# yaramohamadi/Pairwise_Sample_Optimization

Measured on AMD Instinct MI355X. Metric: PSO train-step imgs/sec (paired 1024² SDXL) at 1/2/4/8 MI355X, higher is better.
Workload: dtype bf16; 1 GPU; C2: SDXL-Turbo PSO train step, LoRA r=32 grads, 2 pairs/GPU/micro-step, gas 2, 2-step sampler (T=1); global_batch=4, seq_len=4096, resolution=1024, parallelism=dp1, launch=eager

## Files before the change

### include/pso_amd.h

```cpp
#ifndef PSO_AMD_H
#define PSO_AMD_H

#include <stddef.h>
#include <stdint.h>

#ifdef __cplusplus
extern "C" {
#endif

#define PSO_ABI_VERSION 1

#define PSO_OK 0
#define PSO_ERR_ARG 1
#define PSO_ERR_HIP 2
#define PSO_ERR_UNSUPPORTED 3

#define PSO_F32 0
#define PSO_BF16 1
#define PSO_F16 2
#define PSO_U8 2

#define PSO_MODE_TURBO 0
#define PSO_MODE_DMD 1
#define PSO_MODE_DMD_F16 2
// ... 120 lines not shown
                      long sdq_b, void* dk, long lddk, long sdk_b, void* dv, long lddv, long sdv_b, void* ws,
                      size_t ws_bytes, void* stream);

int pso_geglu_fwd(long M, int F, const void* in, long ldi, void* out, long ldo, void* stream);
int pso_geglu_bwd(long M, int F, const void* in, long ldi, const void* dout, long lddo, void* din, long lddi,
                  void* stream);
int pso_silu(long n, const void* x, void* y, void* stream);
int pso_timestep_embedding(int n, int dim, const float* t, void* out, long ldo, int out_col, void* stream);
int pso_transpose(int R, int Rp, int C, const void* in, long ldi, void* out, long ldo, void* stream);
int pso_im2col3(int B, int H, int W, int C, const void* in, void* out, int Kp, void* stream);

int pso_colsum_acc(long M, int N, const void* x, long ldx, long rows_per_group, float* out, long ldo, void* stream);
int pso_layer_norm_dparam(int M, int C, const void* x, long ldx, const void* dy, long lddy, const float* stats,
                          float* dgamma, float* dbeta, void* stream);
size_t pso_colsum_acc_ws_bytes(long M, int N, long rows_per_group);
int pso_colsum_acc_ws(long M, int N, const void* x, long ldx, long rows_per_group, float* out, long ldo, void* ws,
                      size_t ws_bytes, void* stream);
size_t pso_layer_norm_dparam_ws_bytes(int M, int C);
int pso_layer_norm_dparam_ws(int M, int C, const void* x, long ldx, const void* dy, long lddy, const float* stats,
                             float* dgamma, float* dbeta, void* ws, size_t ws_bytes, void* stream);
int pso_im2col_conv(int mode, int B, const void* src1, int C1, const void* src2, int C2, int H, int W, int Ho, int Wo,
                    int stride, int pad, void* out, long ldo, void* stream);
int pso_sumpool2(int B, int H, int W, int C, const void* in, const void* dadd, void* out, void* stream);
int pso_axpby(long n, float a, const void* x, float b, const void* z, void* y, void* stream);
int pso_cast_f32_bf16(long n, const float* x, float scale, void* y, void* stream);
int pso_cast_bf16_f32(long n, const void* x, float* y, void* stream);
int pso_conv_weight_t(int Co, int ks, int Ci, int flip, const void* w, void* wt, void* stream);
int pso_transpose_batched(int n, const void* descs, int max_r, int max_c, void* stream);
int pso_lora_pack(int n, const void* descs, long max_items, float scale, void* stream);
int pso_lora_grad_fold(int n, const void* descs, long max_items, void* stream);
int pso_transpose_multi(int n, const void* descs, int total_tiles, void* stream);
int pso_gather_rows(long n, long row_bytes, const void* src, const int64_t* idx, void* dst, void* stream);
int pso_nchw_to_nhwc(int B, int C, int Cp, long HW, const void* src, int src_dtype, float scale, void* dst,
                     void* stream);
int pso_softmax_rows(int M, int N, void* x, long ld, void* stream);
int pso_nhwc_to_nchw(int B, int C, long HW, const void* src, void* dst, int dst_dtype, void* stream);
int pso_concat_channels(long npix, int C1, const void* x1, int C2, const void* x2, void* out, void* stream);
int pso_split_channels(long npix, int C1, int C2, const void* in, void* y1, void* y2, const void* add2,
                       void* stream);

size_t pso_grad_clip_ws_bytes(long n);
int pso_grad_clip_coef(long n, const float* grad, float grad_scale, float max_norm, float* out_norm_coef, void* ws,
                       size_t ws_bytes, void* stream);
int pso_adamw_step(long n, float* param, const float* grad, float* exp_avg, float* exp_avg_sq, float lr, float beta1,
                   float beta2, float eps, float weight_decay, int step, float grad_scale, const float* clip_coef,
                   void* stream);
size_t pso_adamw8bit_blocks(long n);
void pso_adamw8bit_maps(float* signed_map, float* unsigned_map);
int pso_adamw8bit_step(long n, float* param, const float* grad, uint8_t* exp_avg_q, uint8_t* exp_avg_sq_q,
                       float* absmax_m, float* absmax_v, float lr, float beta1, float beta2, float eps,
                       float weight_decay, int step, float grad_scale, const float* clip_coef, void* stream);
int pso_adamw8bit_step_bf16(long n, float* param, void* param_bf16, const float* grad, uint8_t* exp_avg_q,
                            uint8_t* exp_avg_sq_q, float* absmax_m, float* absmax_v, float lr, float beta1, float beta2,
                            float eps, float weight_decay, int step, float grad_scale, const float* clip_coef,
                            void* stream);
int pso_adamw8bit_step_blocks(long n, int nblk, const long* desc, float* param, void* param_bf16, const float* grad,
                              uint8_t* exp_avg_q, uint8_t* exp_avg_sq_q, float* absmax_m, float* absmax_v,
                              float* exp_avg_32, float* exp_avg_sq_32, float lr, float beta1, float beta2, float eps,
                              float weight_decay, int step, float grad_scale, const float* clip_coef, void* stream);
int pso_adamw8bit_step_blocks_zero_grad(long n, int nblk, const long* desc, float* param, void* param_bf16,
                                        float* grad, uint8_t* exp_avg_q, uint8_t* exp_avg_sq_q, float* absmax_m,
                                        float* absmax_v, float* exp_avg_32, float* exp_avg_sq_32, float lr,
// ... 76 lines not shown
```

### pairwise_sample_optimization_amd/_lib.py

```python
import ctypes
import os

import torch

_HERE = os.path.dirname(os.path.abspath(__file__))
KNOBS = os.environ.get("PSO_LIB", "") == "knobs"
F16 = os.environ.get("PSO_LIB", "") == "f16"
LIB_PATH = os.environ.get("PSO_LIB_PATH") or os.path.join(
    _HERE, "libpso_amd_knobs.so" if KNOBS else "libpso_amd_f16.so" if F16 else "libpso_amd.so")

PSO_F32 = 0
PSO_BF16 = 1
PSO_F16 = 2
ELEM_DTYPE = torch.float16 if F16 else torch.bfloat16
ELEM_CODE = PSO_F16 if F16 else PSO_BF16
MODE_TURBO = 0
MODE_DMD = 1
MODE_DMD_F16 = 2
MODE_DMD_BF16 = 3
COEF_STRIDE = 8
AMP_WORDS = 16
(AMP_SCALE, AMP_INV_SCALE, AMP_FOUND_INF, AMP_GROWTH_TRACKER, AMP_STEP, AMP_SKIPPED, AMP_NORM, AMP_CLIP_COEF,
 AMP_GRAD_MUL, AMP_BC1, AMP_BC2_SQRT, AMP_C1, AMP_C2) = range(13)
AMP_INT_WORDS = (AMP_FOUND_INF, AMP_GROWTH_TRACKER, AMP_STEP, AMP_SKIPPED)
# ... 68 lines not shown
    "pso_group_norm_ws_bytes": (csz, [ci, ci, ci]),
    "pso_group_norm_fwd": (ci, [ci, ci, ci, ci, cf, vp, vp, vp, ci, vp, vp, vp, csz, vp]),
    "pso_group_norm_bwd": (ci, [ci, ci, ci, ci, vp, vp, vp, vp, vp, ci, vp, vp, vp, vp, ci, vp, csz, vp]),
    "pso_layer_norm_fwd": (ci, [ci, ci, cf, vp, cl, vp, vp, vp, cl, vp, vp]),
    "pso_layer_norm_bwd": (ci, [ci, ci, vp, cl, vp, cl, vp, vp, vp, cl, vp, cl, vp]),
    "pso_attention_fwd": (ci, [ci, ci, ci, ci, vp, cl, cl, vp, cl, cl, vp, cl, cl, cf, vp, cl, cl, vp, vp]),
    "pso_attention_bwd_ws_bytes": (csz, [ci, ci, ci, ci]),
    "pso_attention_bwd": (ci, [ci, ci, ci, ci, vp, cl, cl, vp, cl, cl, vp, cl, cl, vp, cl, cl, vp, vp, cl, cl, cf,
                               vp, cl, cl, vp, cl, cl, vp, cl, cl, vp, csz, vp]),
    "pso_geglu_fwd": (ci, [cl, ci, vp, cl, vp, cl, vp]),
    "pso_geglu_bwd": (ci, [cl, ci, vp, cl, vp, cl, vp, cl, vp]),
    "pso_silu": (ci, [cl, vp, vp, vp]),
    "pso_timestep_embedding": (ci, [ci, ci, vp, vp, cl, ci, vp]),
    "pso_transpose": (ci, [ci, ci, ci, vp, cl, vp, cl, vp]),
    "pso_im2col3": (ci, [ci, ci, ci, ci, vp, vp, ci, vp]),
    "pso_colsum_acc": (ci, [cl, ci, vp, cl, cl, vp, cl, vp]),
    "pso_layer_norm_dparam": (ci, [ci, ci, vp, cl, vp, cl, vp, vp, vp, vp]),
    "pso_colsum_acc_ws_bytes": (csz, [cl, ci, cl]),
    "pso_colsum_acc_ws": (ci, [cl, ci, vp, cl, cl, vp, cl, vp, csz, vp]),
    "pso_layer_norm_dparam_ws_bytes": (csz, [ci, ci]),
    "pso_layer_norm_dparam_ws": (ci, [ci, ci, vp, cl, vp, cl, vp, vp, vp, vp, csz, vp]),
    "pso_im2col_conv": (ci, [ci, ci, vp, ci, vp, ci, ci, ci, ci, ci, ci, ci, vp, cl, vp]),
    "pso_sumpool2": (ci, [ci, ci, ci, ci, vp, vp, vp, vp]),
    "pso_axpby": (ci, [cl, cf, vp, cf, vp, vp, vp]),
    "pso_cast_f32_bf16": (ci, [cl, vp, cf, vp, vp]),
    "pso_cast_bf16_f32": (ci, [cl, vp, vp, vp]),
    "pso_conv_weight_t": (ci, [ci, ci, ci, ci, vp, vp, vp]),
    "pso_concat_channels": (ci, [cl, ci, vp, ci, vp, vp, vp]),
    "pso_nchw_to_nhwc": (ci, [ci, ci, ci, cl, vp, ci, cf, vp, vp]),
    "pso_softmax_rows": (ci, [ci, ci, vp, cl, vp]),
    "pso_grad_clip_ws_bytes": (csz, [cl]),
    "pso_transpose_batched": (ci, [ci, vp, ci, ci, vp]),
    "pso_transpose_multi": (ci, [ci, vp, ci, vp]),
    "pso_lora_pack": (ci, [ci, vp, cl, cf, vp]),
    "pso_lora_grad_fold": (ci, [ci, vp, cl, vp]),
    "pso_gather_rows": (ci, [cl, cl, vp, vp, vp, vp]),
    "pso_grad_clip_coef": (ci, [cl, vp, cf, cf, vp, vp, csz, vp]),
    "pso_adamw_step": (ci, [cl, vp, vp, vp, vp, cf, cf, cf, cf, cf, ci, cf, vp, vp]),
    "pso_adamw8bit_blocks": (csz, [cl]),
    "pso_adamw8bit_maps": (None, [vp, vp]),
    "pso_adamw8bit_step": (ci, [cl, vp, vp, vp, vp, vp, vp, cf, cf, cf, cf, cf, ci, cf, vp, vp]),
    "pso_adamw8bit_step_bf16": (ci, [cl, vp, vp, vp, vp, vp, vp, vp, cf, cf, cf, cf, cf, ci, cf, vp, vp]),
    "pso_adamw8bit_step_blocks": (ci, [cl, ci, vp, vp, vp, vp, vp, vp, vp, vp, vp, vp, cf, cf, cf, cf, cf, ci, cf,
                                       vp, vp]),
    "pso_adamw8bit_step_blocks_zero_grad": (ci, [cl, ci, vp, vp, vp, vp, vp, vp, vp, vp, vp, vp, cf, cf, cf, cf, cf,
                                                 ci, cf, vp, vp]),
    "pso_amp_unscale_clip": (ci, [cl, vp, cf, cf, cf, cf, vp, vp, csz, vp]),
    "pso_amp_update": (ci, [vp, cf, cf, ci, vp]),
    "pso_adamw_step_amp": (ci, [cl, vp, vp, vp, vp, cf, cf, cf, cf, cf, vp, vp]),
    "pso_adamw8bit_step_blocks_amp": (ci, [cl, ci, vp, vp, vp, vp, vp, vp, vp, vp, vp, vp, cf, cf, cf, cf, cf, vp,
                                           vp]),
# ... 114 lines not shown
```

### pairwise_sample_optimization_amd/csrc/elementwise.hip

```cpp
#include "common.h"

__device__ __forceinline__ void unpack8e(uint4 v, float* f) {
  const uint32_t w[4] = {v.x, v.y, v.z, v.w};
#pragma unroll
  for (int i = 0; i < 4; ++i) {
    f[2 * i] = bf2f(w[i] & 0xffff);
    f[2 * i + 1] = bf2f(w[i] >> 16);
  }
}
__device__ __forceinline__ uint4 pack8e(const float* f) {
  return make_uint4(pack2bf(f[0], f[1]), pack2bf(f[2], f[3]), pack2bf(f[4], f[5]), pack2bf(f[6], f[7]));
}

static int grid_for(long n, int per_thread = 1) {
  long g = (n / per_thread + 255) / 256;
  if (g > 8192) g = 8192;
  return (int)(g < 1 ? 1 : g);
}

#define GRID_STRIDE(i, n) for (long i = blockIdx.x * (long)blockDim.x + threadIdx.x; i < (n); i += (long)gridDim.x * blockDim.x)


__global__ void geglu_fwd_kernel(long M, int F, const bf16_t* __restrict__ in, long ldi, bf16_t* __restrict__ out,
                                 long ldo) {
// ... 128 lines not shown
  const int C8 = C / 8;
  GRID_STRIDE(v, (long)B * H * W * C8) {
    const long pix = v / C8;
    const int c = (int)(v - pix * C8) * 8;
    const int b = (int)(pix / ((long)H * W));
    const int rem = (int)(pix - (long)b * H * W);
    const int y = rem / W, x = rem - y * W;
    float acc[8] = {0, 0, 0, 0, 0, 0, 0, 0};
#pragma unroll
    for (int dy = 0; dy < 2; ++dy)
#pragma unroll
      for (int dx = 0; dx < 2; ++dx) {
        float a[8];
        unpack8e(*reinterpret_cast<const uint4*>(in + (((long)b * 2 * H + 2 * y + dy) * 2 * W + 2 * x + dx) * C + c), a);
#pragma unroll
        for (int j = 0; j < 8; ++j) acc[j] += a[j];
      }
    if (dadd) {
      float a[8];
      unpack8e(*reinterpret_cast<const uint4*>(dadd + pix * C + c), a);
#pragma unroll
      for (int j = 0; j < 8; ++j) acc[j] += a[j];
    }
    *reinterpret_cast<uint4*>(out + pix * C + c) = pack8e(acc);
  }
}

__global__ void axpby_kernel(long n8, float a, const bf16_t* __restrict__ x, float b, const bf16_t* __restrict__ z,
                             bf16_t* __restrict__ y) {
  GRID_STRIDE(v, n8) {
    float p[8], q[8];
    unpack8e(*reinterpret_cast<const uint4*>(x + v * 8), p);
    if (z) unpack8e(*reinterpret_cast<const uint4*>(z + v * 8), q);
#pragma unroll
    for (int j = 0; j < 8; ++j) p[j] = a * p[j] + (z ? b * q[j] : 0.f);
    *reinterpret_cast<uint4*>(y + v * 8) = pack8e(p);
  }
}

__global__ void cast_f32_bf16_kernel(long n, const float* __restrict__ x, float scale, bf16_t* __restrict__ y) {
  long done = 0;
  if (((reinterpret_cast<uintptr_t>(x) | reinterpret_cast<uintptr_t>(y)) & 15) == 0) {
    done = n & ~7L;
    GRID_STRIDE(v, n >> 3) {
      const float4 a = reinterpret_cast<const float4*>(x)[2 * v], b = reinterpret_cast<const float4*>(x)[2 * v + 1];
      reinterpret_cast<uint4*>(y)[v] = make_uint4(pack2bf(a.x * scale, a.y * scale), pack2bf(a.z * scale, a.w * scale),
// ... 39 lines not shown
      for (int e = 0; e < 8; ++e) tile[r][c + e] = (co < Co && ci + e < Ci) ? src[e] : (bf16_t)0;
    }
  }
  __syncthreads();
  const int lx = t & 63, ly = t >> 6;
  for (int i = ly; i < 64; i += 4) {
    const int ci = ci0 + i, co = co0 + lx;
    if (ci < Ci && co < Co) wt[((long)ci * ks * ks + tap2) * Co + co] = tile[lx][i];
  }
}

__global__ void concat_kernel(long npix, int C1, const bf16_t* __restrict__ x1, int C2, const bf16_t* __restrict__ x2,
                              bf16_t* __restrict__ out) {
  const int C8 = (C1 + C2) / 8, c18 = C1 / 8;
  GRID_STRIDE(v, npix * C8) {
    const long p = v / C8;
    const int ch = (int)(v - p * C8);
    const uint4 val = ch < c18 ? *reinterpret_cast<const uint4*>(x1 + p * C1 + ch * 8)
                               : *reinterpret_cast<const uint4*>(x2 + p * C2 + (ch - c18) * 8);
    *reinterpret_cast<uint4*>(out + v * 8) = val;
  }
}

__global__ void split_kernel(long npix, int C1, int C2, const bf16_t* __restrict__ in, bf16_t* __restrict__ y1,
                             bf16_t* __restrict__ y2, const bf16_t* __restrict__ add2) {
  const int C8 = (C1 + C2) / 8, c18 = C1 / 8;
  GRID_STRIDE(v, npix * C8) {
    const long p = v / C8;
    const int ch = (int)(v - p * C8);
    const uint4 val = *reinterpret_cast<const uint4*>(in + v * 8);
    if (ch < c18) {
      *reinterpret_cast<uint4*>(y1 + p * C1 + ch * 8) = val;
    } else {
      bf16_t* o = y2 + p * C2 + (ch - c18) * 8;
      if (add2) {
        float a[8], b[8];
        unpack8e(val, a);
        unpack8e(*reinterpret_cast<const uint4*>(add2 + p * C2 + (ch - c18) * 8), b);
#pragma unroll
        for (int j = 0; j < 8; ++j) a[j] += b[j];
        *reinterpret_cast<uint4*>(o) = pack8e(a);
      } else {
        *reinterpret_cast<uint4*>(o) = val;
      }
    }
  }
// ... 120 lines not shown
                     void* stream) {
  PSO_DTYPE_CHECK(src_dtype, "pso_nchw_to_nhwc");
  PSO_ARG_CHECK(src && dst && Cp >= C, "pso_nchw_to_nhwc: bad args");
  nchw_to_nhwc_kernel<<<grid_for((long)B * Cp * HW), 256, 0, (hipStream_t)stream>>>(
      B, C, Cp, HW, src, src_dtype == PSO_F32, scale, (bf16_t*)dst);
  return pso_check_launch("pso_nchw_to_nhwc");
}

int pso_nhwc_to_nchw(int B, int C, long HW, const void* src, void* dst, int dst_dtype, void* stream) {
  PSO_DTYPE_CHECK(dst_dtype, "pso_nhwc_to_nchw");
  PSO_ARG_CHECK(src && dst, "pso_nhwc_to_nchw: bad args");
  nhwc_to_nchw_kernel<<<grid_for((long)B * C * HW), 256, 0, (hipStream_t)stream>>>(B, C, HW, (const bf16_t*)src,
                                                                                  dst, dst_dtype == PSO_F32);
  return pso_check_launch("pso_nhwc_to_nchw");
}

int pso_concat_channels(long npix, int C1, const void* x1, int C2, const void* x2, void* out, void* stream) {
  PSO_ARG_CHECK(C1 % 8 == 0 && C2 % 8 == 0 && x1 && x2 && out, "pso_concat_channels: C %% 8");
  concat_kernel<<<grid_for(npix * (C1 + C2) / 8), 256, 0, (hipStream_t)stream>>>(
      npix, C1, (const bf16_t*)x1, C2, (const bf16_t*)x2, (bf16_t*)out);
  return pso_check_launch("pso_concat_channels");
}

int pso_split_channels(long npix, int C1, int C2, const void* in, void* y1, void* y2, const void* add2,
                       void* stream) {
  PSO_ARG_CHECK(C1 % 8 == 0 && C2 % 8 == 0 && in && y1 && y2, "pso_split_channels: C %% 8");
  split_kernel<<<grid_for(npix * (C1 + C2) / 8), 256, 0, (hipStream_t)stream>>>(
      npix, C1, C2, (const bf16_t*)in, (bf16_t*)y1, (bf16_t*)y2, (const bf16_t*)add2);
  return pso_check_launch("pso_split_channels");
}

int pso_geglu_fwd(long M, int F, const void* in, long ldi, void* out, long ldo, void* stream) {
  PSO_ARG_CHECK(F % 8 == 0 && ldi % 8 == 0 && ldo % 8 == 0 && in && out, "pso_geglu_fwd: bad args");
  geglu_fwd_kernel<<<grid_for(M * (F / 8)), 256, 0, (hipStream_t)stream>>>(M, F, (const bf16_t*)in, ldi,
                                                                          (bf16_t*)out, ldo);
  return pso_check_launch("pso_geglu_fwd");
}

int pso_geglu_bwd(long M, int F, const void* in, long ldi, const void* dout, long lddo, void* din, long lddi,
                  void* stream) {
  PSO_ARG_CHECK(F % 8 == 0 && ldi % 8 == 0 && lddo % 8 == 0 && lddi % 8 == 0 && in && dout && din,
                "pso_geglu_bwd: bad args");
  geglu_bwd_kernel<<<grid_for(M * (F / 8)), 256, 0, (hipStream_t)stream>>>(M, F, (const bf16_t*)in, ldi,
                                                                          (const bf16_t*)dout, lddo, (bf16_t*)din,
                                                                          lddi);
  return pso_check_launch("pso_geglu_bwd");
// ... 19 lines not shown
}

int pso_transpose(int R, int Rp, int C, const void* in, long ldi, void* out, long ldo, void* stream) {
  PSO_ARG_CHECK(in && out && Rp >= R, "pso_transpose: bad args");
  dim3 grid(cdiv(C, 64), cdiv(Rp, 64));
  transpose_kernel<<<grid, 256, 0, (hipStream_t)stream>>>(R, Rp, C, (const bf16_t*)in, ldi, (bf16_t*)out, ldo);
  return pso_check_launch("pso_transpose");
}

int pso_im2col3(int B, int H, int W, int C, const void* in, void* out, int Kp, void* stream) {
  PSO_ARG_CHECK(Kp >= 9 * C && in && out, "pso_im2col3: Kp < 9C");
  im2col3_kernel<<<grid_for((long)B * H * W * Kp), 256, 0, (hipStream_t)stream>>>(B, H, W, C, (const bf16_t*)in, 0,
                                                                                  (bf16_t*)out, Kp);
  return pso_check_launch("pso_im2col3");
}

int pso_sumpool2(int B, int H, int W, int C, const void* in, const void* dadd, void* out, void* stream) {
  PSO_ARG_CHECK(C % 8 == 0 && in && out, "pso_sumpool2: C %% 8");
  sumpool2_kernel<<<grid_for((long)B * H * W * C / 8), 256, 0, (hipStream_t)stream>>>(
      B, H, W, C, (const bf16_t*)in, (const bf16_t*)dadd, (bf16_t*)out);
  return pso_check_launch("pso_sumpool2");
}

int pso_axpby(long n, float a, const void* x, float b, const void* z, void* y, void* stream) {
  PSO_ARG_CHECK(n % 8 == 0 && x && y, "pso_axpby: n %% 8");
  axpby_kernel<<<grid_for(n / 8), 256, 0, (hipStream_t)stream>>>(n / 8, a, (const bf16_t*)x, b, (const bf16_t*)z,
                                                                 (bf16_t*)y);
  return pso_check_launch("pso_axpby");
}

int pso_cast_f32_bf16(long n, const float* x, float scale, void* y, void* stream) {
  cast_f32_bf16_kernel<<<grid_for(n, 8), 256, 0, (hipStream_t)stream>>>(n, x, scale, (bf16_t*)y);
  return pso_check_launch("pso_cast_f32_bf16");
}

int pso_cast_bf16_f32(long n, const void* x, float* y, void* stream) {
  cast_bf16_f32_kernel<<<grid_for(n, 8), 256, 0, (hipStream_t)stream>>>(n, (const bf16_t*)x, y);
  return pso_check_launch("pso_cast_bf16_f32");
}

int pso_conv_weight_t(int Co, int ks, int Ci, int flip, const void* w, void* wt, void* stream) {
  conv_weight_t_kernel<<<dim3(cdiv(Ci, 64), cdiv(Co, 64), ks * ks), 256, 0, (hipStream_t)stream>>>(
      Co, ks, Ci, flip, (const bf16_t*)w, (bf16_t*)wt);
  return pso_check_launch("pso_conv_weight_t");
}

// ... 2 lines not shown
```

### pairwise_sample_optimization_amd/kernels.py

```python
import ctypes
import math
import os

import torch

from . import _lib
from ._lib import check, lib, ptr, require_cuda, stream_ptr, dtype_code, PSO_BF16, PSO_F32

CONV_NORMAL, CONV_UP2, CONV_T2 = 1, 2, 3
ELEM = _lib.ELEM_DTYPE

PROFILE = None


def _prof_begin():
    if PROFILE is None:
        return None
    e0 = torch.cuda.Event(enable_timing=True)
    e0.record()
    return e0


def _prof_end(e0, flops, nbytes=0.0, tag=None):
    if e0 is not None:
# ... 293 lines not shown
        self.pending = {}


def conv2d(x, weight, *, x2=None, mode=CONV_NORMAL, stride=1, pad=None, out_hw=None, bias=None, rowbias=None,
           resid=None, a2=None, w2=None, alpha=1.0, out=None, out_dtype=ELEM, accumulate=False):
    require_cuda(x, weight)
    B, H, W, C1 = x.shape
    C2 = x2.shape[3] if x2 is not None else 0
    Cout, ks, ks2, Ct = weight.shape
    assert ks == ks2 and Ct == C1 + C2 and x.is_contiguous() and weight.is_contiguous()
    if pad is None:
        pad = ks // 2
    if out_hw is None:
        if mode == CONV_UP2:
            out_hw = (2 * H, 2 * W)
        elif mode == CONV_T2:
            out_hw = (2 * H, 2 * W)
        else:
            out_hw = ((H + 2 * pad - ks) // stride + 1, (W + 2 * pad - ks) // stride + 1)
    Ho, Wo = out_hw
    if out is None:
        out = torch.empty((B, Ho, Wo, Cout), device=x.device, dtype=out_dtype)
    K2 = a2.shape[1] if a2 is not None else 0
    o2 = out.view(B * Ho * Wo, -1) if out.is_contiguous() else None
    ldo = Cout if o2 is None else o2.stride(0)
    key = ("conv", B, Ho, Wo, Cout, ks * ks * Ct, K2)
    wsb = _GEMM_WS.get(key)
    if wsb is None:
        wsb = _GEMM_WS[key] = int(lib().pso_conv2d_ws_bytes(B, Ho, Wo, Cout, ks * ks * Ct, K2))
    args = (mode, B, ptr(x), C1, ptr(x2), C2, H, W, Ho, Wo, ks, stride, pad, ptr(weight), Cout,
            ptr(a2), _row_stride(a2) if a2 is not None else 0, K2,
            ptr(w2), _row_stride(w2) if w2 is not None else 0, float(alpha), ptr(bias),
            ptr(rowbias), rowbias.stride(0) if rowbias is not None else 0,
            ptr(resid), Cout if resid is not None else 0, ptr(out), ldo, dtype_code(out), int(accumulate))
    e0 = _prof_begin()
    if wsb:
        ws = torch.empty(wsb, device=x.device, dtype=torch.uint8)
        check(lib().pso_conv2d_ws(*args, ptr(ws), wsb, stream_ptr()), "pso_conv2d_ws")
    else:
        check(lib().pso_conv2d(*args, stream_ptr()), "pso_conv2d")
    _prof_end(e0, 2.0 * B * Ho * Wo * Cout * (ks * ks * (C1 + C2) + K2),
              2.0 * (B * H * W * (C1 + C2) + Cout * ks * ks * (C1 + C2) + B * Ho * Wo * K2 + Cout * K2)
              + out.element_size() * B * Ho * Wo * Cout, ("conv", mode, B, H, W, C1, C2, Cout, ks, stride, K2))
    return out


def step_logprob(mode, sample, eps, coef, prev=None, noise=None, noise_shared=False):
    require_cuda(sample, eps, coef, prev, noise)
# ... 270 lines not shown
        _row_stride(out)
        _TRANSPOSE_BATCH.append((x, out))
        return out
    check(lib().pso_transpose(R, Rp, C, ptr(x), _row_stride(x), ptr(out), _row_stride(out), stream_ptr()),
          "pso_transpose")
    return out


def im2col3(x, kp):
    B, H, W, C = x.shape
    out = torch.empty((B * H * W, kp), device=x.device, dtype=x.dtype)
    check(lib().pso_im2col3(B, H, W, C, ptr(x.contiguous()), ptr(out), kp, stream_ptr()), "pso_im2col3")
    return out


def sumpool2(x, dadd=None):
    B, H2, W2, C = x.shape
    out = torch.empty((B, H2 // 2, W2 // 2, C), device=x.device, dtype=x.dtype)
    check(lib().pso_sumpool2(B, H2 // 2, W2 // 2, C, ptr(x.contiguous()), ptr(dadd), ptr(out), stream_ptr()),
          "pso_sumpool2")
    return out


def axpby(a, x, b=0.0, z=None, out=None):
    out = torch.empty_like(x) if out is None else out
    check(lib().pso_axpby(x.numel(), float(a), ptr(x.contiguous()), float(b),
                          ptr(z.contiguous()) if z is not None else None, ptr(out), stream_ptr()), "pso_axpby")
    return out


_FULLGRAD_ATOMIC = os.environ.get("PSO_FULLGRAD_ATOMIC", "0") == "1"
_STREAM_WS = {}


def _stream_ws(nbytes, device):
    key = (device.index, torch.cuda.current_stream(device).cuda_stream)
    ws = _STREAM_WS.get(key)
    if ws is None or ws.numel() < nbytes:
        ws = _STREAM_WS[key] = torch.empty(max(int(nbytes * 1.25), 1 << 16), device=device, dtype=torch.uint8)
    return ws


def colsum_acc(x, out, rows_per_group=None):
    M, N = x.shape
    rpg = M if rows_per_group is None else rows_per_group
    if _FULLGRAD_ATOMIC:
# ... 44 lines not shown


def cast_bf16_f32(x, out=None):
    out = torch.empty(x.shape, device=x.device, dtype=torch.float32) if out is None else out
    check(lib().pso_cast_bf16_f32(x.numel(), ptr(x.contiguous()), ptr(out), stream_ptr()), "pso_cast_bf16_f32")
    return out


def conv_weight_t(w, flip):
    Co, ks, _, Ci = w.shape
    out = torch.empty((Ci, ks, ks, Co), device=w.device, dtype=w.dtype)
    check(lib().pso_conv_weight_t(Co, ks, Ci, int(flip), ptr(w.contiguous()), ptr(out), stream_ptr()),
          "pso_conv_weight_t")
    return out


def concat_channels(x1, x2):
    C1, C2 = x1.shape[-1], x2.shape[-1]
    out = torch.empty(x1.shape[:-1] + (C1 + C2,), device=x1.device, dtype=x1.dtype)
    npix = x1.numel() // C1
    check(lib().pso_concat_channels(npix, C1, ptr(x1.contiguous()), C2, ptr(x2.contiguous()), ptr(out),
                                    stream_ptr()), "pso_concat_channels")
    return out


def split_channels(x, C1, add2=None):
    C = x.shape[-1]
    C2 = C - C1
    y1 = torch.empty(x.shape[:-1] + (C1,), device=x.device, dtype=x.dtype)
    y2 = torch.empty(x.shape[:-1] + (C2,), device=x.device, dtype=x.dtype)
    npix = x.numel() // C
    check(lib().pso_split_channels(npix, C1, C2, ptr(x.contiguous()), ptr(y1), ptr(y2),
                                   ptr(add2.contiguous()) if add2 is not None else None, stream_ptr()),
          "pso_split_channels")
    return y1, y2


def nchw_to_nhwc(x, pad_to=None, scale=1.0):
    B, C, H, W = x.shape
    Cp = pad_to or C
    out = torch.empty((B, H, W, Cp), device=x.device, dtype=ELEM)
    check(lib().pso_nchw_to_nhwc(B, C, Cp, H * W, ptr(x.contiguous()), dtype_code(x), float(scale), ptr(out),
                                 stream_ptr()), "pso_nchw_to_nhwc")
    return out


# ... 450 lines not shown
```

### pairwise_sample_optimization_amd/unet.py

```python
import math
import os
from dataclasses import dataclass, field, replace
from types import SimpleNamespace

import torch
import torch.nn as nn

from . import _lib
from . import kernels as K

ELEM = _lib.ELEM_DTYPE
TN_BATCH = os.environ.get("PSO_TN_BATCH", "1") != "0"


@dataclass
class UNetConfig:
    in_channels: int = 4
    out_channels: int = 4
    block_out_channels: tuple = (320, 640, 1280)
    layers_per_block: int = 2
    transformer_layers_per_block: tuple = (1, 2, 10)
    down_has_attn: tuple = (False, True, True)
    head_dim: int = 64
    cross_attention_dim: int = 2048
# ... 740 lines not shown
        self.wt_int = K.transpose(self.w_int)
        self.out.prepare()

    def _remap(self):
        return {"net.0.proj": self.proj, "net.2": self.out}


class Transformer2DModel(nn.Module):

    def __init__(self, C, depth, cross_dim, groups):
        super().__init__()
        self.C, self.groups = C, groups
        self.norm = Norm(C)
        self.proj_in = Linear(C, C)
        self.transformer_blocks = nn.ModuleList([BasicTransformerBlock(C, cross_dim) for _ in range(depth)])
        self.proj_out = Linear(C, C)

    def prepare(self):
        self.proj_in.prepare()
        self.proj_out.prepare()
        for b in self.transformer_blocks:
            b.prepare()

    def fwd(self, x, rt, path):
        B, H, W, C = x.shape
        xn, st = K.group_norm_fwd(x, self.norm.weight, self.norm.bias, self.groups, 1e-6, False)
        h = K.gemm(xn.view(-1, C), self.proj_in.weight, bias=self.proj_in.bias)
        if rt.save:
            rt.saved.append({"x": rt.pol(x), "st": rt.pol(st), "xn": xn.view(-1, C) if rt.fg is not None else None})
        for i, blk in enumerate(self.transformer_blocks):
            h = blk.fwd(h, rt, f"{path}.transformer_blocks.{i}")
        if rt.save and rt.fg is not None:
            rt.saved.append({"hout": h})
        return K.gemm(h, self.proj_out.weight, bias=self.proj_out.bias, resid=x.view(-1, C)).view(B, H, W, C)

    def bwd(self, dy, rt, path, need_dx=True):
        B, H, W, C = dy.shape
        d2 = dy.view(-1, C)
        fg = rt.fg
        if fg is not None:
            _lin_dw(fg, self.proj_out, d2, rt.saved.pop()["hout"], rt)
        dh = K.gemm(d2, self.proj_out.wt)
        for i in reversed(range(len(self.transformer_blocks))):
            dh = self.transformer_blocks[i].bwd(dh, rt.saved.pop(), rt, f"{path}.transformer_blocks.{i}",
                                                need_dx=need_dx or i > 0)
        sv = rt.saved.pop()
        if not need_dx:
            return None
        dn = K.gemm(dh, self.proj_in.wt).view(B, H, W, C)
        if fg is not None:
            _lin_dw(fg, self.proj_in, dh, sv["xn"], rt)
            return K.group_norm_bwd(sv["x"], dn, sv["st"], self.norm.weight, self.norm.bias, False, dadd=dy,
                                    dgamma=fg.g(self.norm.weight), dbeta=fg.g(self.norm.bias), accumulate=True)
        return K.group_norm_bwd(sv["x"], dn, sv["st"], self.norm.weight, self.norm.bias, False, dadd=dy)


class ResnetBlock2D(nn.Module):
    def __init__(self, cin, cout, groups, eps, temb_dim):
        super().__init__()
        self.cin, self.cout, self.groups, self.eps = cin, cout, groups, eps
        self.norm1 = Norm(cin)
        self.conv1 = Conv2d(cin, cout, 3)
        self.time_emb_proj = Linear(temb_dim, cout) if temb_dim else None
        self.norm2 = Norm(cout)
        self.conv2 = Conv2d(cout, cout, 3)
        self.conv_shortcut = Conv2d(cin, cout, 1) if cin != cout else None

    def prepare(self):
        self.conv1.prepare()
        self.conv2.prepare()
        if self.conv_shortcut is not None:
            self.conv_shortcut.prepare()

    def fwd(self, x, rt, temb=None):
        h1, st1 = K.group_norm_fwd(x, self.norm1.weight, self.norm1.bias, self.groups, self.eps, True)
        c1 = K.conv2d(h1, self.conv1.w_nhwc, bias=self.conv1.bias, rowbias=temb)
        h2, st2 = K.group_norm_fwd(c1, self.norm2.weight, self.norm2.bias, self.groups, self.eps, True)
        if self.conv_shortcut is not None:
            B, H, W, _ = x.shape
            sc = K.gemm(x.view(-1, self.cin), self.conv_shortcut.w_mat, bias=self.conv_shortcut.bias)
            sc = sc.view(B, H, W, self.cout)
        else:
            sc = x
        out = K.conv2d(h2, self.conv2.w_nhwc, bias=self.conv2.bias, resid=sc)
        if rt.save:
            sv = {"x": rt.pol(x), "st1": rt.pol(st1), "c1": rt.pol(c1), "st2": rt.pol(st2)}
            if rt.fg is not None:
                sv.update(h1=h1, h2=h2)
            rt.saved.append(sv)
        return out

    def bwd(self, dout, rt):
        sv = rt.saved.pop()
        fg = rt.fg
        B, H, W, _ = dout.shape
        dh2 = K.conv2d(dout, self.conv2.w_dx)
        if fg is not None:
            _conv_dw(fg, self.conv2, dout.view(-1, self.cout), sv["h2"], rt, K.im2col_conv)
            dc1 = K.group_norm_bwd(sv["c1"], dh2, sv["st2"], self.norm2.weight, self.norm2.bias, True,
                                   dgamma=fg.g(self.norm2.weight), dbeta=fg.g(self.norm2.bias), accumulate=True)
            dc2 = dc1.view(-1, self.cout)
            _conv_dw(fg, self.conv1, dc2, sv["h1"], rt, K.im2col_conv)
            K.colsum_acc(dc2, rt.dtemb[:, self._temb_off:self._temb_off + self.cout], rows_per_group=H * W)
        else:
            dc1 = K.group_norm_bwd(sv["c1"], dh2, sv["st2"], self.norm2.weight, self.norm2.bias, True)
        dh1 = K.conv2d(dc1, self.conv1.w_dx)
        if self.conv_shortcut is not None:
# ... 23 lines not shown
        self.conv.prepare()

    def fwd(self, x, rt):
        if rt.save:
            rt.saved.append({"hw": x.shape[1:3], "x": x if rt.fg is not None else None})
        return K.conv2d(x, self.conv.w_nhwc, stride=2, bias=self.conv.bias)

    def bwd(self, dy, rt):
        sv = rt.saved.pop()
        if rt.fg is not None:
            _conv_dw(rt.fg, self.conv, dy.reshape(-1, self.conv.cout), sv["x"], rt,
                     lambda x: K.im2col_conv(x, stride=2))
        return K.conv2d(dy, self.conv.w_dx, mode=K.CONV_T2, out_hw=tuple(sv["hw"]))


class Upsample2D(nn.Module):
    def __init__(self, C):
        super().__init__()
        self.conv = Conv2d(C, C, 3)

    def prepare(self):
        self.conv.prepare()

    def fwd(self, x, rt):
        if rt.save and rt.fg is not None:
            rt.saved.append({"x": x})
        return K.conv2d(x, self.conv.w_nhwc, mode=K.CONV_UP2, bias=self.conv.bias)

    def bwd(self, dy, rt):
        if rt.fg is not None:
            _conv_dw(rt.fg, self.conv, dy.reshape(-1, self.conv.cout), rt.saved.pop()["x"], rt,
                     lambda x: K.im2col_conv(x, mode=K.CONV_UP2))
        du = K.conv2d(dy, self.conv.w_dx)
        return K.sumpool2(du)


class _Block(nn.Module):

    def __init__(self):
        super().__init__()


class TimestepEmbedding(nn.Module):
    def __init__(self, fin, dim):
        super().__init__()
        self.linear_1 = Linear(fin, dim)
        self.linear_2 = Linear(dim, dim)


class _Output(SimpleNamespace):
    pass


class UNet2DConditionModel(nn.Module):
    def __init__(self, config: UNetConfig = None):
        super().__init__()
        cfg = config or UNetConfig.sdxl()
# ... 316 lines not shown
            self.prepare()
        B = x.shape[0]
        lora_on = self.lora is not None and self._adapters_enabled
        encf = enc.to(ELEM).reshape(B * enc.shape[1], enc.shape[2]).contiguous()
        rt = self._runtime(B, encf, save, lora_on)
        temb_all = self._embed(timestep, time_ids, text_embeds, B, x.device)
        tb = lambda m: temb_all[:, m._temb_off:m._temb_off + m.cout]
        _, H, W, _ = x.shape
        cols = K.im2col3(x, self.conv_in.kp)
        h = K.gemm(cols, self.conv_in.w_col, bias=self.conv_in.bias).view(B, H, W, -1)
        skips = [h]
        i0, j0 = self._first_attn
        full = rt.fg is not None
        if full and paired_ref:
            raise ValueError("full-UNet training: the reference is a separate frozen UNet, not the adapter-free pass")
        if full:
            rt.emb = self._emb_saved
            rt.cols_in = cols
            i0, j0 = -1, -1
        else:
            rt.save = False
        for i, blk in enumerate(self.down_blocks):
            for j, res in enumerate(blk.resnets):
                if (i, j) == (i0, j0):
                    rt.save = save
                    if paired_ref:
                        dup = lambda t: torch.cat([t, t], 0)
                        h = dup(h)
                        skips = [dup(s_) for s_ in skips]
                        temb_all = dup(temb_all)
                        rt.enc = dup(rt.enc)
                        rt.B = 2 * B
                        rt.paired = True
                h = res.fwd(h, rt, tb(res))
                if hasattr(blk, "attentions"):
                    h = blk.attentions[j].fwd(h, rt, f"down_blocks.{i}.attentions.{j}")
                skips.append(h)
            if hasattr(blk, "downsamplers"):
                h = blk.downsamplers[0].fwd(h, rt)
                skips.append(h)
        m = self.mid_block
        h = m.resnets[0].fwd(h, rt, tb(m.resnets[0]))
        h = m.attentions[0].fwd(h, rt, "mid_block.attentions.0")
        h = m.resnets[1].fwd(h, rt, tb(m.resnets[1]))
        for i, blk in enumerate(self.up_blocks):
            for j, res in enumerate(blk.resnets):
                s = skips.pop()
                hc = K.concat_channels(h, s)
                if rt.save:
                    rt.saved.append({"c1": h.shape[-1]})
                h = res.fwd(hc, rt, tb(res))
                if hasattr(blk, "attentions"):
                    h = blk.attentions[j].fwd(h, rt, f"up_blocks.{i}.attentions.{j}")
            if hasattr(blk, "upsamplers"):
                h = blk.upsamplers[0].fwd(h, rt)
        hn, st = K.group_norm_fwd(h, self.conv_norm_out.weight, self.conv_norm_out.bias, self.cfg.norm_num_groups,
                                  self.cfg.norm_eps, True)
        out = K.conv2d(hn, self.conv_out.w_nhwc, bias=self.conv_out.bias)
        if save:
            rt.saved.append({"h": rt.pol(h), "st": rt.pol(st), "hn": hn if full else None})
        rt.B = B
        rt.enc = rt.pol(rt.enc)
        rt.paired = False
        return out, rt

    def backward_nhwc(self, dout, rt):
        B = dout.shape[0]
        sv = rt.saved.pop()
        fg = rt.fg
        _, H, W, _ = dout.shape
        cols = K.im2col3(dout.contiguous(), self.conv_out.kp_dx)
        dhn = K.gemm(cols, self.conv_out.w_dx_col).view(B, H, W, -1)
        if fg is not None:
            rt.dtemb = torch.zeros((B, self._temb_n), device=dout.device, dtype=torch.float32)
            co = self.conv_out.cout
            dy8 = torch.zeros((B * H * W, 8), device=dout.device, dtype=ELEM)
            dy8[:, :co] = dout.reshape(-1, co)
            _conv_dw(fg, self.conv_out, dy8, sv["hn"], rt, K.im2col_conv)
# ... 160 lines not shown
```

Before: 39.26 imgs/s.

## Drop up-block concats, broadcast skips, and use box-sum strided conv for upsample dx

Up-block resnet, attention and upsampler outputs are now written straight into the left half of a preallocated concat buffer, and the skip tensor is copied into the right half. A new copy_cols kernel does that copy and broadcasts single-batch skips across the paired batch by modulo indexing, so the full concat and the eager duplication of the skip list are no longer needed. The upsampler input-gradient changes from a full-resolution conv followed by sumpool2 to a 2x2 box sum followed by a stride-2 conv, which cuts that conv's work by about 4x. The first resnet at the paired split point now runs before duplication with saving disabled, which alters what is saved for backward. That reordering and the strided output writes are risks to correctness.

```diff
diff --git a/include/pso_amd.h b/include/pso_amd.h
--- a/include/pso_amd.h
+++ b/include/pso_amd.h
@@ -166,6 +166,7 @@
 int pso_im2col_conv(int mode, int B, const void* src1, int C1, const void* src2, int C2, int H, int W, int Ho, int Wo,
                     int stride, int pad, void* out, long ldo, void* stream);
 int pso_sumpool2(int B, int H, int W, int C, const void* in, const void* dadd, void* out, void* stream);
+int pso_box2_sum(int B, int H2, int W2, int C, const void* in, void* out, void* stream);
 int pso_axpby(long n, float a, const void* x, float b, const void* z, void* y, void* stream);
 int pso_cast_f32_bf16(long n, const float* x, float scale, void* y, void* stream);
 int pso_cast_bf16_f32(long n, const void* x, float* y, void* stream);
@@ -182,6 +183,7 @@
 int pso_concat_channels(long npix, int C1, const void* x1, int C2, const void* x2, void* out, void* stream);
 int pso_split_channels(long npix, int C1, int C2, const void* in, void* y1, void* y2, const void* add2,
                        void* stream);
+int pso_copy_cols(long npix, long npix_src, int C, const void* src, void* out, long ldo, void* stream);
 
 size_t pso_grad_clip_ws_bytes(long n);
 int pso_grad_clip_coef(long n, const float* grad, float grad_scale, float max_norm, float* out_norm_coef, void* ws,
diff --git a/pairwise_sample_optimization_amd/_lib.py b/pairwise_sample_optimization_amd/_lib.py
--- a/pairwise_sample_optimization_amd/_lib.py
+++ b/pairwise_sample_optimization_amd/_lib.py
@@ -114,11 +114,13 @@
     "pso_layer_norm_dparam_ws": (ci, [ci, ci, vp, cl, vp, cl, vp, vp, vp, vp, csz, vp]),
     "pso_im2col_conv": (ci, [ci, ci, vp, ci, vp, ci, ci, ci, ci, ci, ci, ci, vp, cl, vp]),
     "pso_sumpool2": (ci, [ci, ci, ci, ci, vp, vp, vp, vp]),
+    "pso_box2_sum": (ci, [ci, ci, ci, ci, vp, vp, vp]),
     "pso_axpby": (ci, [cl, cf, vp, cf, vp, vp, vp]),
     "pso_cast_f32_bf16": (ci, [cl, vp, cf, vp, vp]),
     "pso_cast_bf16_f32": (ci, [cl, vp, vp, vp]),
     "pso_conv_weight_t": (ci, [ci, ci, ci, ci, vp, vp, vp]),
     "pso_concat_channels": (ci, [cl, ci, vp, ci, vp, vp, vp]),
+    "pso_copy_cols": (ci, [cl, cl, ci, vp, vp, cl, vp]),
     "pso_nchw_to_nhwc": (ci, [ci, ci, ci, cl, vp, ci, cf, vp, vp]),
     "pso_softmax_rows": (ci, [ci, ci, vp, cl, vp]),
     "pso_grad_clip_ws_bytes": (csz, [cl]),
diff --git a/pairwise_sample_optimization_amd/csrc/elementwise.hip b/pairwise_sample_optimization_amd/csrc/elementwise.hip
--- a/pairwise_sample_optimization_amd/csrc/elementwise.hip
+++ b/pairwise_sample_optimization_amd/csrc/elementwise.hip
@@ -174,6 +174,32 @@
 #pragma unroll
       for (int j = 0; j < 8; ++j) acc[j] += a[j];
     }
+    *reinterpret_cast<uint4*>(out + pix * C + c) = pack8e(acc);
+  }
+}
+
+__global__ void box2_sum_kernel(int B, int H2, int W2, int C, const bf16_t* __restrict__ in,
+                                bf16_t* __restrict__ out) {
+  const int C8 = C / 8, Ho = H2 + 1, Wo = W2 + 1;
+  GRID_STRIDE(v, (long)B * Ho * Wo * C8) {
+    const long pix = v / C8;
+    const int c = (int)(v - pix * C8) * 8;
+    const int b = (int)(pix / ((long)Ho * Wo));
+    const int rem = (int)(pix - (long)b * Ho * Wo);
+    const int y = rem / Wo, x = rem - y * Wo;
+    float acc[8] = {0, 0, 0, 0, 0, 0, 0, 0};
+#pragma unroll
+    for (int dy = -1; dy <= 0; ++dy)
+#pragma unroll
+      for (int dx = -1; dx <= 0; ++dx) {
+        const int iy = y + dy, ix = x + dx;
+        if ((unsigned)iy < (unsigned)H2 && (unsigned)ix < (unsigned)W2) {
+          float a[8];
+          unpack8e(*reinterpret_cast<const uint4*>(in + (((long)b * H2 + iy) * W2 + ix) * C + c), a);
+#pragma unroll
+          for (int j = 0; j < 8; ++j) acc[j] += a[j];
+        }
+      }
     *reinterpret_cast<uint4*>(out + pix * C + c) = pack8e(acc);
   }
 }
@@ -259,6 +285,17 @@
   }
 }
 
+__global__ void copy_cols_kernel(long npix, long npix_src, int C, const bf16_t* __restrict__ src,
+                                 bf16_t* __restrict__ out, long ldo) {
+  const int C8 = C / 8;
+  GRID_STRIDE(v, npix * C8) {
+    const long p = v / C8;
+    const int c = (int)(v - p * C8) * 8;
+    const long ps = p < npix_src ? p : p % npix_src;
+    *reinterpret_cast<uint4*>(out + p * ldo + c) = *reinterpret_cast<const uint4*>(src + ps * C + c);
+  }
+}
+
 __global__ void split_kernel(long npix, int C1, int C2, const bf16_t* __restrict__ in, bf16_t* __restrict__ y1,
                              bf16_t* __restrict__ y2, const bf16_t* __restrict__ add2) {
   const int C8 = (C1 + C2) / 8, c18 = C1 / 8;
@@ -425,6 +462,16 @@
   return pso_check_launch("pso_concat_channels");
 }
 
+int pso_copy_cols(long npix, long npix_src, int C, const void* src, void* out, long ldo, void* stream) {
+  PSO_ARG_CHECK(npix > 0 && npix_src > 0 && npix % npix_src == 0 && C > 0 && C % 8 == 0 && ldo >= C && ldo % 8 == 0 &&
+                    src && out,
+                "pso_copy_cols: needs C %% 8, ldo %% 8, ldo >= C and npix a multiple of npix_src");
+  PSO_ARG_CHECK(((uintptr_t)src % 16) == 0 && ((uintptr_t)out % 16) == 0, "pso_copy_cols: 16-B alignment");
+  copy_cols_kernel<<<grid_for(npix * C / 8), 256, 0, (hipStream_t)stream>>>(npix, npix_src, C, (const bf16_t*)src,
+                                                                            (bf16_t*)out, ldo);
+  return pso_check_launch("pso_copy_cols");
+}
+
 int pso_split_channels(long npix, int C1, int C2, const void* in, void* y1, void* y2, const void* add2,
                        void* stream) {
   PSO_ARG_CHECK(C1 % 8 == 0 && C2 % 8 == 0 && in && y1 && y2, "pso_split_channels: C %% 8");
@@ -490,6 +537,14 @@
   return pso_check_launch("pso_sumpool2");
 }
 
+int pso_box2_sum(int B, int H2, int W2, int C, const void* in, void* out, void* stream) {
+  PSO_ARG_CHECK(B > 0 && H2 > 0 && W2 > 0 && C > 0 && C % 8 == 0 && in && out, "pso_box2_sum: C %% 8");
+  PSO_ARG_CHECK(((uintptr_t)in % 16) == 0 && ((uintptr_t)out % 16) == 0, "pso_box2_sum: 16-B alignment");
+  box2_sum_kernel<<<grid_for((long)B * (H2 + 1) * (W2 + 1) * C / 8), 256, 0, (hipStream_t)stream>>>(
+      B, H2, W2, C, (const bf16_t*)in, (bf16_t*)out);
+  return pso_check_launch("pso_box2_sum");
+}
+
 int pso_axpby(long n, float a, const void* x, float b, const void* z, void* y, void* stream) {
   PSO_ARG_CHECK(n % 8 == 0 && x && y, "pso_axpby: n %% 8");
   axpby_kernel<<<grid_for(n / 8), 256, 0, (hipStream_t)stream>>>(n / 8, a, (const bf16_t*)x, b, (const bf16_t*)z,
diff --git a/pairwise_sample_optimization_amd/kernels.py b/pairwise_sample_optimization_amd/kernels.py
--- a/pairwise_sample_optimization_amd/kernels.py
+++ b/pairwise_sample_optimization_amd/kernels.py
@@ -339,8 +339,10 @@
     if out is None:
         out = torch.empty((B, Ho, Wo, Cout), device=x.device, dtype=out_dtype)
     K2 = a2.shape[1] if a2 is not None else 0
-    o2 = out.view(B * Ho * Wo, -1) if out.is_contiguous() else None
-    ldo = Cout if o2 is None else o2.stride(0)
+    ldo = Cout if out.is_contiguous() else out.stride(2)
+    assert tuple(out.shape) == (B, Ho, Wo, Cout) and ldo >= Cout and all(
+        n == 1 or s == want for n, s, want in zip(out.shape, out.stride(), (Ho * Wo * ldo, Wo * ldo, ldo, 1))), \
+        "conv2d: out must be NHWC with one pixel pitch"
     key = ("conv", B, Ho, Wo, Cout, ks * ks * Ct, K2)
     wsb = _GEMM_WS.get(key)
     if wsb is None:
@@ -657,6 +659,21 @@
     return out
 
 
+def box2_sum(x):
+    require_cuda(x)
+    B, H2, W2, C = x.shape
+    assert x.is_contiguous()
+    out = torch.empty((B, H2 + 1, W2 + 1, C), device=x.device, dtype=x.dtype)
+    check(lib().pso_box2_sum(B, H2, W2, C, ptr(x), ptr(out), stream_ptr()), "pso_box2_sum")
+    return out
+
+
+def upsample2_conv_dx(dy, w_dx):
+    B, H2, W2, _ = dy.shape
+    assert H2 % 2 == 0 and W2 % 2 == 0
+    return conv2d(box2_sum(dy), w_dx, stride=2, pad=0, out_hw=(H2 // 2, W2 // 2))
+
+
 def axpby(a, x, b=0.0, z=None, out=None):
     out = torch.empty_like(x) if out is None else out
     check(lib().pso_axpby(x.numel(), float(a), ptr(x.contiguous()), float(b),
@@ -747,6 +764,22 @@
     check(lib().pso_concat_channels(npix, C1, ptr(x1.contiguous()), C2, ptr(x2.contiguous()), ptr(out),
                                     stream_ptr()), "pso_concat_channels")
     return out
+
+
+def cat_buffer(like, B, H, W, C1, C2):
+    hc = torch.empty((B, H, W, C1 + C2), device=like.device, dtype=like.dtype)
+    return hc, hc[..., :C1]
+
+
+def copy_cols(src, hc, C1):
+    require_cuda(src, hc)
+    B, H, W, Ct = hc.shape
+    C2 = Ct - C1
+    assert hc.is_contiguous() and src.is_contiguous() and src.dtype == hc.dtype
+    assert tuple(src.shape[1:]) == (H, W, C2) and B % src.shape[0] == 0 and C1 % 8 == 0
+    check(lib().pso_copy_cols(B * H * W, src.shape[0] * H * W, C2, ptr(src), ptr(hc[..., C1:]), Ct,
+                              stream_ptr()), "pso_copy_cols")
+    return hc
 
 
 def split_channels(x, C1, add2=None):
diff --git a/pairwise_sample_optimization_amd/unet.py b/pairwise_sample_optimization_amd/unet.py
--- a/pairwise_sample_optimization_amd/unet.py
+++ b/pairwise_sample_optimization_amd/unet.py
@@ -786,7 +786,7 @@
         for b in self.transformer_blocks:
             b.prepare()
 
-    def fwd(self, x, rt, path):
+    def fwd(self, x, rt, path, out=None):
         B, H, W, C = x.shape
         xn, st = K.group_norm_fwd(x, self.norm.weight, self.norm.bias, self.groups, 1e-6, False)
         h = K.gemm(xn.view(-1, C), self.proj_in.weight, bias=self.proj_in.bias)
@@ -796,6 +796,10 @@
             h = blk.fwd(h, rt, f"{path}.transformer_blocks.{i}")
         if rt.save and rt.fg is not None:
             rt.saved.append({"hout": h})
+        if out is not None:
+            K.gemm(h, self.proj_out.weight, bias=self.proj_out.bias, resid=x.view(-1, C),
+                   out=out.as_strided((B * H * W, C), (out.stride(2), 1)))
+            return out
         return K.gemm(h, self.proj_out.weight, bias=self.proj_out.bias, resid=x.view(-1, C)).view(B, H, W, C)
 
     def bwd(self, dy, rt, path, need_dx=True):
@@ -836,7 +840,7 @@
         if self.conv_shortcut is not None:
             self.conv_shortcut.prepare()
 
-    def fwd(self, x, rt, temb=None):
+    def fwd(self, x, rt, temb=None, out=None):
         h1, st1 = K.group_norm_fwd(x, self.norm1.weight, self.norm1.bias, self.groups, self.eps, True)
         c1 = K.conv2d(h1, self.conv1.w_nhwc, bias=self.conv1.bias, rowbias=temb)
         h2, st2 = K.group_norm_fwd(c1, self.norm2.weight, self.norm2.bias, self.groups, self.eps, True)
@@ -846,7 +850,7 @@
             sc = sc.view(B, H, W, self.cout)
         else:
             sc = x
-        out = K.conv2d(h2, self.conv2.w_nhwc, bias=self.conv2.bias, resid=sc)
+        out = K.conv2d(h2, self.conv2.w_nhwc, bias=self.conv2.bias, resid=sc, out=out)
         if rt.save:
             sv = {"x": rt.pol(x), "st1": rt.pol(st1), "c1": rt.pol(c1), "st2": rt.pol(st2)}
             if rt.fg is not None:
@@ -916,17 +920,16 @@
     def prepare(self):
         self.conv.prepare()
 
-    def fwd(self, x, rt):
+    def fwd(self, x, rt, out=None):
         if rt.save and rt.fg is not None:
             rt.saved.append({"x": x})
-        return K.conv2d(x, self.conv.w_nhwc, mode=K.CONV_UP2, bias=self.conv.bias)
+        return K.conv2d(x, self.conv.w_nhwc, mode=K.CONV_UP2, bias=self.conv.bias, out=out)
 
     def bwd(self, dy, rt):
         if rt.fg is not None:
             _conv_dw(rt.fg, self.conv, dy.reshape(-1, self.conv.cout), rt.saved.pop()["x"], rt,
                      lambda x: K.im2col_conv(x, mode=K.CONV_UP2))
-        du = K.conv2d(dy, self.conv.w_dx)
-        return K.sumpool2(du)
+        return K.upsample2_conv_dx(dy, self.conv.w_dx)
 
 
 class _Block(nn.Module):
@@ -1289,17 +1292,16 @@
             rt.save = False
         for i, blk in enumerate(self.down_blocks):
             for j, res in enumerate(blk.resnets):
+                h = res.fwd(h, rt, tb(res))
                 if (i, j) == (i0, j0):
                     rt.save = save
                     if paired_ref:
                         dup = lambda t: torch.cat([t, t], 0)
                         h = dup(h)
-                        skips = [dup(s_) for s_ in skips]
                         temb_all = dup(temb_all)
                         rt.enc = dup(rt.enc)
                         rt.B = 2 * B
                         rt.paired = True
-                h = res.fwd(h, rt, tb(res))
                 if hasattr(blk, "attentions"):
                     h = blk.attentions[j].fwd(h, rt, f"down_blocks.{i}.attentions.{j}")
                 skips.append(h)
@@ -1309,18 +1311,31 @@
         m = self.mid_block
         h = m.resnets[0].fwd(h, rt, tb(m.resnets[0]))
         h = m.attentions[0].fwd(h, rt, "mid_block.attentions.0")
-        h = m.resnets[1].fwd(h, rt, tb(m.resnets[1]))
+
+        def cat_for(c1):
+            s = skips[-1]
+            return K.cat_buffer(s, rt.B, s.shape[1], s.shape[2], c1, s.shape[3])
+
+        hc, left = cat_for(m.resnets[1].cout)
+        m.resnets[1].fwd(h, rt, tb(m.resnets[1]), out=left)
+        n_up = len(self.up_blocks)
         for i, blk in enumerate(self.up_blocks):
+            attn, ups, nres = hasattr(blk, "attentions"), hasattr(blk, "upsamplers"), len(blk.resnets)
             for j, res in enumerate(blk.resnets):
-                s = skips.pop()
-                hc = K.concat_channels(h, s)
+                c1 = left.shape[-1]
+                K.copy_cols(skips.pop(), hc, c1)
                 if rt.save:
-                    rt.saved.append({"c1": h.shape[-1]})
-                h = res.fwd(hc, rt, tb(res))
-                if hasattr(blk, "attentions"):
-                    h = blk.attentions[j].fwd(h, rt, f"up_blocks.{i}.attentions.{j}")
-            if hasattr(blk, "upsamplers"):
-                h = blk.upsamplers[0].fwd(h, rt)
+                    rt.saved.append({"c1": c1})
+                x, nxt, left = hc, None, None
+                if j + 1 < nres or (not ups and i + 1 < n_up):
+                    nxt, left = cat_for(res.cout)
+                h = res.fwd(x, rt, tb(res), out=None if attn else left)
+                if attn:
+                    h = blk.attentions[j].fwd(h, rt, f"up_blocks.{i}.attentions.{j}", out=left)
+                hc = nxt
+            if ups:
+                hc, left = cat_for(blk.upsamplers[0].conv.cout)
+                blk.upsamplers[0].fwd(h, rt, out=left)
         hn, st = K.group_norm_fwd(h, self.conv_norm_out.weight, self.conv_norm_out.bias, self.cfg.norm_num_groups,
                                   self.cfg.norm_eps, True)
         out = K.conv2d(hn, self.conv_out.w_nhwc, bias=self.conv_out.bias)
```

After: 39.57 imgs/s, median of 6. Within noise of the previous version (+0.8%).
